# gvanhorn38/multibox

Measured on AMD Instinct MI355X. Metric: images/sec (299x299, 5-AR priors) train, higher is better.
Workload: dtype bf16; 1 GPU; full train step: Inception-ResNet-v2 + multibox heads fwd, on-device matching+loss, bwd, RMSProp+EMA; 299x299, k=5 (P=646), BATCH_SIZE=64/GPU, MAX_NUM_BBOXES=13; global_batch=64, parallelism=dp1, hip_graph=True

## Files before the change

multibox_amd/csrc/nnops.hip:

```cpp
#include "common.h"
#include <stdlib.h>
#include <string.h>

namespace {

__device__ __forceinline__ int xcd_logical(int bid, int nblk) {
  const int xcd = bid & 7, q = nblk >> 3, r = nblk & 7;
  return (xcd < r ? xcd * (q + 1) : r * (q + 1) + (xcd - r) * q) + (bid >> 3);
}
inline int xcd_rows_on() { static const int v = mbx_env_int("MBX_XCD_ROWS", 0); return v; }


typedef __attribute__((ext_vector_type(4))) unsigned int u32x4;
typedef __attribute__((ext_vector_type(2))) unsigned int u32x2;
constexpr int kT = 256;

__device__ __forceinline__ float bf2f(unsigned h) { return __uint_as_float(h << 16); }
__device__ __forceinline__ unsigned f2bf(float f) { return (unsigned)__builtin_bit_cast(unsigned short, (__bf16)f); }
__device__ __forceinline__ unsigned pack2bf(float lo, float hi) {
  typedef float pk_f32x2 __attribute__((ext_vector_type(2)));
  typedef __bf16 pk_bf16x2 __attribute__((ext_vector_type(2)));
  return __builtin_bit_cast(unsigned, __builtin_convertvector(pk_f32x2{lo, hi}, pk_bf16x2));
}
__device__ __forceinline__ float relu_f(float x) {
// ... 710 lines not shown
    const int e = threadIdx.x % C2, p = threadIdx.x / C2;
    float t[1];
    if (p < np) {
      ob_sum_cols<1, 16>(sred + p * C2 + e, 0, 1, np * C2, (rpi - p + np - 1) / np, t);
      part[p * C2 + e] = t[0];
    }
    __syncthreads();
    if (threadIdx.x < C2) {
      ob_sum_cols<1, 16>(part + threadIdx.x, 0, 1, C2, np, t);
      atomicAdd(acc + threadIdx.x, t[0]);
    }
  } else if (rpi > 8) ob_reduce_wide<1, 16>(sred, C2, rpi, acc);
  else if (rpi > 4) ob_reduce_wide<2, 8>(sred, C2, rpi, acc);
  else if (rpi > 2) ob_reduce_wide<4, 4>(sred, C2, rpi, acc);
  else if (rpi > 1) ob_reduce_wide<8, 2>(sred, C2, rpi, acc);
  else ob_reduce_wide<16, 1>(sred, C2, rpi, acc);
  asm volatile("s_waitcnt vmcnt(0) lgkmcnt(0)" ::: "memory");
  __syncthreads();
  if (threadIdx.x == 0) {
    const unsigned G = gridDim.x, b = blockIdx.x;
    const unsigned sub = b % kObSub, n_sub = (G - sub + kObSub - 1) / kObSub, n_top = G < kObSub ? G : kObSub;
    s_timeout = 0;
    bool last = ((fault & 1) && b == 0) ? false : atomicAdd(ctl + kObLine * (1 + sub), 1u) == n_sub - 1;
    if (last) last = atomicAdd(ctl + kObLine * (1 + kObSub), 1u) == n_top - 1;
    if (last) {
      for (int r = 0; r < kObRel; ++r)
        __hip_atomic_store(ctl + kObLine * (2 + kObSub + r), 1u, __ATOMIC_RELAXED, __HIP_MEMORY_SCOPE_AGENT);
    } else {
      const unsigned* rel = ctl + kObLine * (2 + kObSub + b % kObRel);
      unsigned spins = 0;
      while (ld_agent(rel) == 0u) {
        __builtin_amdgcn_s_sleep(MBX_OB_SLEEP);
        if (++spins > spin_limit) {
          ctl[1] = 1u; s_timeout = 1;
          if (step_poison) atomicAdd(step_poison, 1.0f);
          break;
        }
      }
    }
    if (b == 0) ctl[0] = G;
  }
  __syncthreads();
  for (int e = threadIdx.x; e < 2 * C; e += kObT) {
    float t = 0.f;
#pragma unroll
    for (int sl = 0; sl < kObSlots; ++sl) t += ld_agent(ws + (size_t)sl * 2 * C + e);
    sred[e] = t;
  }
  __syncthreads();
  float m1[8], m2[8], t1[8];
  const float poison = s_timeout ? __builtin_nanf("") : 0.f;
  {
    const float* tot = sred + (active ? c : 0);
    u32x4 p0 = *reinterpret_cast<const u32x4*>(tot), p1 = *reinterpret_cast<const u32x4*>(tot + 4);
    u32x4 q0 = *reinterpret_cast<const u32x4*>(tot + C), q1 = *reinterpret_cast<const u32x4*>(tot + C + 4);
    asm volatile("" : "+v"(p0), "+v"(p1), "+v"(q0), "+v"(q1));
#pragma unroll
    for (int j = 0; j < 4; ++j) {
      t1[j] = __uint_as_float(p0[j]); t1[4 + j] = __uint_as_float(p1[j]);
      m2[j] = __uint_as_float(q0[j]); m2[4 + j] = __uint_as_float(q1[j]);
    }
  }
#pragma unroll
  for (int j = 0; j < 8; ++j) {
    t1[j] = (active ? t1[j] : 0.f) + poison;
    m1[j] = t1[j] * inv_M;
    m2[j] = (active ? m2[j] : 0.f) * inv_M;
  }
  if (blockIdx.x == 0 && rr == 0 && dbeta) {
#pragma unroll
    for (int j = 0; j < 8; ++j) atomicAdd(dbeta + c + j, t1[j]);
  }
#pragma unroll
  for (int i = 0; i < NV; ++i) {
    const int lr = rr + i * rpi;
    const bool ok = active && lr < nrows;
    asm volatile("" : "+v"(vg[i]), "+v"(vy[i]));
    float g[8], yy[8], o[8];
    unpack8(vg[i], g);
    unpack8(vy[i], yy);
#pragma unroll
    for (int j = 0; j < 8; ++j) {
      const float xh = (yy[j] - mu[j]) * rs[j];
      const float gj = (!RELU || xh + be[j] > 0.f) ? g[j] : 0.f;
      o[j] = rs[j] * (gj - m1[j] - xh * m2[j]);
    }
    ob_store16(dr, ok ? (unsigned)((lr * C + c) * 2) : kPast, pack8(o));
    asm volatile("" ::: "memory");
  }
}

template <int KK, int SS>
__global__ void __launch_bounds__(kT)
maxpool_fwd_kernel(const unsigned short* __restrict__ x, long long xs, int ldx, int N, int H, int W, int C, int k_,
                   int stride_, unsigned short* __restrict__ y, long long ys, int ldy, int Ho, int Wo,
                   unsigned char* __restrict__ argmax) {
  const int k = KK ? KK : k_, stride = SS ? SS : stride_;
  const int C8 = C >> 3;
  const unsigned total = (unsigned)N * Ho * Wo * C8;
  for (unsigned i = blockIdx.x * kT + threadIdx.x; i < total; i += gridDim.x * kT) {
    unsigned t = i / (unsigned)C8;
    const int c = (int)(i - t * C8) << 3;
    const unsigned t2 = t / (unsigned)Wo;
    const int ow = (int)(t - t2 * Wo);
    const int n = (int)(t2 / (unsigned)Ho);
    const int oh = (int)(t2 - (unsigned)n * Ho);
    float best[8];
    unsigned arg[8];
#pragma unroll
    for (int j = 0; j < 8; ++j) { best[j] = -INFINITY; arg[j] = 0; }
    if constexpr (KK > 0) {
      u32x4 v[KK * KK];
#pragma unroll
      for (int r = 0; r < KK; ++r)
#pragma unroll
        for (int s = 0; s < KK; ++s) {
          const int h = oh * stride + r, w = ow * stride + s;
          v[r * KK + s] = (h < H && w < W) ? ld8(x + n * xs + ((long long)h * W + w) * ldx + c) : u32x4{0u, 0u, 0u, 0u};
        }
#pragma unroll
      for (int r = 0; r < KK; ++r)
#pragma unroll
        for (int s = 0; s < KK; ++s) {
          const int h = oh * stride + r, w = ow * stride + s;
          if (h >= H || w >= W) continue;
          float f[8];
          unpack8(v[r * KK + s], f);
#pragma unroll
          for (int j = 0; j < 8; ++j)
            if (f[j] > best[j]) { best[j] = f[j]; arg[j] = r * KK + s; }
        }
    } else {
      for (int r = 0; r < k; ++r)
        for (int s = 0; s < k; ++s) {
          const int h = oh * stride + r, w = ow * stride + s;
          if (h >= H || w >= W) continue;
          float f[8];
          unpack8(ld8(x + n * xs + ((long long)h * W + w) * ldx + c), f);
#pragma unroll
          for (int j = 0; j < 8; ++j)
            if (f[j] > best[j]) { best[j] = f[j]; arg[j] = r * k + s; }
        }
    }
    st8(y + n * ys + ((long long)oh * Wo + ow) * ldy + c, pack8(best));
    if (argmax) {
      u32x2 av;
      av.x = arg[0] | (arg[1] << 8) | (arg[2] << 16) | (arg[3] << 24);
      av.y = arg[4] | (arg[5] << 8) | (arg[6] << 16) | (arg[7] << 24);
      *reinterpret_cast<u32x2*>(argmax + (((long long)n * Ho + oh) * Wo + ow) * C + c) = av;
    }
  }
}

__global__ void __launch_bounds__(kT)
bn_apply_maxpool3s2_kernel(const unsigned short* __restrict__ y, int N, int H, int W, int C, const float* __restrict__ mean,
                           const float* __restrict__ rstd, const float* __restrict__ beta, int relu,
                           unsigned short* __restrict__ p, long long ps, int ldp, int Ho, int Wo,
                           unsigned char* __restrict__ argmax) {
  const int C8 = C >> 3;
  const unsigned total = (unsigned)N * Ho * Wo * C8;
  for (unsigned i = blockIdx.x * kT + threadIdx.x; i < total; i += gridDim.x * kT) {
    unsigned t = i / (unsigned)C8;
    const int c = (int)(i - t * C8) << 3;
    const unsigned t2 = t / (unsigned)Wo;
    const int ow = (int)(t - t2 * Wo);
    const int n = (int)(t2 / (unsigned)Ho);
    const int oh = (int)(t2 - (unsigned)n * Ho);
    u32x4 v[9];
#pragma unroll
    for (int r = 0; r < 3; ++r)
#pragma unroll
      for (int q = 0; q < 3; ++q)
        v[r * 3 + q] = ld8(y + (((long long)n * H + (oh * 2 + r)) * W + (ow * 2 + q)) * C + c);
    float mu[8], rs[8], be[8], best[8];
    unsigned arg[8];
#pragma unroll
    for (int j = 0; j < 8; ++j) { mu[j] = mean[c + j]; rs[j] = rstd[c + j]; be[j] = beta[c + j]; best[j] = -INFINITY; arg[j] = 0; }
#pragma unroll
    for (int tq = 0; tq < 9; ++tq) {
      float f[8];
      unpack8(v[tq], f);
#pragma unroll
      for (int j = 0; j < 8; ++j) {
        float a = (f[j] - mu[j]) * rs[j] + be[j];
        a = relu ? relu_f(a) : a;
        a = bf2f(f2bf(a));
        if (a > best[j]) { best[j] = a; arg[j] = tq; }
      }
    }
    st8(p + n * ps + ((long long)oh * Wo + ow) * ldp + c, pack8(best));
    if (argmax) {
      u32x2 av;
      av.x = arg[0] | (arg[1] << 8) | (arg[2] << 16) | (arg[3] << 24);
      av.y = arg[4] | (arg[5] << 8) | (arg[6] << 16) | (arg[7] << 24);
      *reinterpret_cast<u32x2*>(argmax + (((long long)n * Ho + oh) * Wo + ow) * C + c) = av;
    }
  }
}

struct PoolSrc { const unsigned short* gy; long long gys; int ld_gy; const unsigned char* argmax; int H, W, Ho, Wo, C, Hb, Wb; };
__device__ __forceinline__ void pool3s2_grad_block(const PoolSrc& p, int n, int a, int b, int c, float (&g)[4][8]) {
  u32x4 gv[4];
  u32x2 av[4];
  bool ok[4];
#pragma unroll
  for (int i = 0; i < 4; ++i) {
    const int oh = a - 1 + (i >> 1), ow = b - 1 + (i & 1);
    const bool v = oh >= 0 && oh < p.Ho && ow >= 0 && ow < p.Wo;
    ok[i] = v;
    const long long o = ((long long)n * p.Ho + (v ? oh : 0)) * p.Wo + (v ? ow : 0);
    av[i] = v ? *reinterpret_cast<const u32x2*>(p.argmax + o * p.C + c) : u32x2{0xffffffffu, 0xffffffffu};
    gv[i] = v ? ld8(p.gy + n * p.gys + ((long long)oh * p.Wo + ow) * p.ld_gy + c) : u32x4{0u, 0u, 0u, 0u};
  }
  float w[4][8];
#pragma unroll
  for (int i = 0; i < 4; ++i) unpack8(gv[i], w[i]);
  (void)ok;
#pragma unroll
  for (int j = 0; j < 8; ++j) {
    unsigned t[4];
#pragma unroll
    for (int i = 0; i < 4; ++i) t[i] = ((j < 4 ? av[i].x : av[i].y) >> (8 * (j & 3))) & 0xffu;
    float p00 = 0.f, p01 = 0.f, p10 = 0.f, p11 = 0.f;
    if (t[0] == 8u) p00 += w[0][j];
    if (t[1] == 6u) p00 += w[1][j];
    if (t[2] == 2u) p00 += w[2][j];
    if (t[3] == 0u) p00 += w[3][j];
    if (t[1] == 7u) p01 += w[1][j];
    if (t[3] == 1u) p01 += w[3][j];
    if (t[2] == 5u) p10 += w[2][j];
    if (t[3] == 3u) p10 += w[3][j];
    if (t[3] == 4u) p11 += w[3][j];
    g[0][j] = bf2f(f2bf(p00)); g[1][j] = bf2f(f2bf(p01)); g[2][j] = bf2f(f2bf(p10)); g[3][j] = bf2f(f2bf(p11));
  }
}

template <bool RELU>
__global__ void __launch_bounds__(kT)
bn_bwd_reduce_pool_kernel(const PoolSrc ps, const unsigned short* __restrict__ y, long long Mb, int C,
                          const float* __restrict__ mean, const float* __restrict__ rstd, const float* __restrict__ beta,
                          int rpi, int rpb, float* __restrict__ partial) {
  extern __shared__ __attribute__((aligned(16))) float sred[];
  const int C8 = C >> 3;
  const int vc = threadIdx.x % C8, rr = threadIdx.x / C8;
  const bool active = rr < rpi;
  const int c = vc << 3;
  float s1[8], s2[8], mu[8], rs[8], be[8];
#pragma unroll
  for (int j = 0; j < 8; ++j) {
    s1[j] = 0.f; s2[j] = 0.f; mu[j] = mean[c + j]; rs[j] = rstd[c + j];
    be[j] = RELU ? beta[c + j] : 0.f;
  }
  const long long r0 = (long long)blockIdx.x * rpb;
  long long r1 = r0 + rpb;
  if (r1 > Mb) r1 = Mb;
  const unsigned HWb = (unsigned)(ps.Hb * ps.Wb);
  if (active)
    for (long long m = r0 + rr; m < r1; m += rpi) {
      const unsigned mu_ = (unsigned)m, n = mu_ / HWb, rem = mu_ - n * HWb, a = rem / (unsigned)ps.Wb, b = rem - a * (unsigned)ps.Wb;
      u32x4 yv[4];
      bool in[4];
#pragma unroll
      for (int q = 0; q < 4; ++q) {
        const int h = 2 * (int)a + (q >> 1), w = 2 * (int)b + (q & 1);
        in[q] = h < ps.H && w < ps.W;
        yv[q] = ld8(y + (((long long)n * ps.H + (h < ps.H ? h : ps.H - 1)) * ps.W + (w < ps.W ? w : ps.W - 1)) * C + c);
      }
      float g[4][8];
      pool3s2_grad_block(ps, (int)n, (int)a, (int)b, c, g);
#pragma unroll
      for (int q = 0; q < 4; ++q) {
        float yy[8];
        unpack8(yv[q], yy);
#pragma unroll
        for (int j = 0; j < 8; ++j) {
          const float xh = (yy[j] - mu[j]) * rs[j];
          const float gj = (in[q] && (!RELU || xh + be[j] > 0.f)) ? g[q][j] : 0.f;
          s1[j] += gj;
          s2[j] += gj * xh;
        }
      }
    }
  if (active) {
    float* o = sred + ((size_t)rr * C8 + vc) * 16;
#pragma unroll
    for (int j = 0; j < 8; ++j) { o[j] = s1[j]; o[8 + j] = s2[j]; }
  }
  __syncthreads();
  if (threadIdx.x < C8) {
#pragma unroll
    for (int j = 0; j < 8; ++j) { s1[j] = 0.f; s2[j] = 0.f; }
    for (int r = 0; r < rpi; ++r) {
      const float* o = sred + ((size_t)r * C8 + threadIdx.x) * 16;
#pragma unroll
      for (int j = 0; j < 8; ++j) { s1[j] += o[j]; s2[j] += o[8 + j]; }
    }
    float* p = partial + ((size_t)blockIdx.x * C + (threadIdx.x << 3)) * 2;
#pragma unroll
    for (int j = 0; j < 8; ++j) { p[2 * j] = s1[j]; p[2 * j + 1] = s2[j]; }
  }
}

template <bool RELU>
__global__ void __launch_bounds__(kT)
bn_bwd_apply_pool_kernel(const PoolSrc ps, const unsigned short* __restrict__ y, long long Mb, int C, long long M,
                         const float* __restrict__ mean, const float* __restrict__ rstd, const float* __restrict__ beta,
                         const float* __restrict__ m12, unsigned short* __restrict__ dy) {
  const int C8 = C >> 3;
  const long long total = Mb * C8;
  const unsigned HWb = (unsigned)(ps.Hb * ps.Wb);
  for (long long i = (long long)blockIdx.x * kT + threadIdx.x; i < total; i += (long long)gridDim.x * kT) {
    const long long m = i / C8;
    const int c = (int)(i - m * C8) << 3;
    const unsigned mu_ = (unsigned)m, n = mu_ / HWb, rem = mu_ - n * HWb, a = rem / (unsigned)ps.Wb, b = rem - a * (unsigned)ps.Wb;
    float g[4][8], mu[8], rs[8], be[8], q1[8], q2[8];
#pragma unroll
    for (int j = 0; j < 8; ++j) {
      mu[j] = mean[c + j]; rs[j] = rstd[c + j]; be[j] = RELU ? beta[c + j] : 0.f; q1[j] = m12[c + j]; q2[j] = m12[C + c + j];
    }
    u32x4 yv[4];
#pragma unroll
    for (int q = 0; q < 4; ++q) {
      const int h = 2 * (int)a + (q >> 1), w = 2 * (int)b + (q & 1);
      yv[q] = ld8(y + (((long long)n * ps.H + (h < ps.H ? h : ps.H - 1)) * ps.W + (w < ps.W ? w : ps.W - 1)) * C + c);
    }
    pool3s2_grad_block(ps, (int)n, (int)a, (int)b, c, g);
#pragma unroll
    for (int q = 0; q < 4; ++q) {
      const int h = 2 * (int)a + (q >> 1), w = 2 * (int)b + (q & 1);
      if (h >= ps.H || w >= ps.W) continue;
      const long long row = ((long long)n * ps.H + h) * ps.W + w;
      float yy[8], o[8];
      unpack8(yv[q], yy);
#pragma unroll
      for (int j = 0; j < 8; ++j) {
        const float xh = (yy[j] - mu[j]) * rs[j];
        const float gj = (!RELU || xh + be[j] > 0.f) ? g[q][j] : 0.f;
        o[j] = rs[j] * (gj - q1[j] - xh * q2[j]);
      }
      st8(dy + row * C + c, pack8(o));
    }
  }
}

template <int KK, int SS>
__global__ void __launch_bounds__(kT)
maxpool_bwd_kernel(const unsigned short* __restrict__ dy, long long dys, int ld_dy,
                   const unsigned char* __restrict__ argmax, int N, int H, int W, int C, int k_, int stride_, int Ho,
// ... 581 lines not shown
extern "C" int mbx_bn_bwd_apply_mapped(const void* da, int ld_da, const void* a, int ld_a, int relu, const void* y, int64_t M,
                                       int C, const float* mean, const float* rstd, const float* beta, const float* m12,
                                       void* dy, const mbx_chan_map* da_map, mbx_stream_t stream) {
  if (!m12 || !dy || !al16(dy) || !bn_bwd_args_ok(da, ld_da, a, ld_a, relu, y, M, C, mean, rstd, beta))
    return MBX_ERR_INVALID_ARG;
  ChanMap cm;
  if (to_chan_map(da_map, C, cm) != MBX_OK || (da_map && da_map->n && a)) return MBX_ERR_INVALID_ARG;
  MBX_ENTER();
#define MBX_BN_APP(MASK)                                                                                            \
  hipLaunchKernelGGL(bn_bwd_apply_kernel<MASK>, dim3(grid_for(M * (C / 8))), dim3(kT), 0, mbx_s(stream), (cus)da,   \
                     ld_da, (cus)a, ld_a, (cus)y, (long long)M, C, mean, rstd, beta, m12, (us)dy, cm)
  if (!relu) MBX_BN_APP(0); else if (a) MBX_BN_APP(1); else MBX_BN_APP(2);
#undef MBX_BN_APP
  MBX_LAUNCH_CHECK();
  return MBX_OK;
}

extern "C" int mbx_bn_bwd_apply_rows(const float* stats, int rows, const void* da, int ld_da, const void* y, int64_t M, int C,
                                     const float* mean, const float* rstd, const float* relu_thr, float* dbeta, void* dy,
                                     const mbx_chan_map* da_map, mbx_stream_t stream) {
  if (!stats || rows <= 0 || rows > 16 || !da || !y || !mean || !rstd || !relu_thr || !dy || M <= 0 || C <= 0 || C % 8 ||
      ld_da % 8 || !al16(da) || !al16(y) || !al16(dy) || !al16(stats))
    return MBX_ERR_INVALID_ARG;
  if (C > kRowsMaxC) return MBX_ERR_UNSUPPORTED;
  ChanMap cm;
  if (to_chan_map(da_map, C, cm) != MBX_OK) return MBX_ERR_INVALID_ARG;
  MBX_ENTER();
  static const int rows_blocks = mbx_env_int("MBX_BN_ROWS_BLOCKS", 1024);
  const int C8 = C / 8, rpi = kT / C8 > 0 ? kT / C8 : 1;
  long long g = (M + rpi - 1) / rpi;
  if (g > rows_blocks) g = rows_blocks;
  hipLaunchKernelGGL(bn_bwd_rows_kernel, dim3((unsigned)g), dim3(kT), (size_t)5 * C * sizeof(float), mbx_s(stream), stats, rows,
                     1.0 / (double)M, (cus)da, ld_da, (cus)y, (long long)M, C, mean, rstd, relu_thr, dbeta, (us)dy, cm);
  MBX_LAUNCH_CHECK();
  return MBX_OK;
}

extern "C" size_t mbx_bn_bwd_onepass_workspace_bytes(int C) {
  return C > 0 ? ((size_t)kObSlots * 2 * C + kObCtlWords) * sizeof(float) : 0;
}

static int ob_groups(int max_workgroups) {
  const int ncu = mbx_cu_count();
  return (max_workgroups > 0 && max_workgroups < ncu) ? max_workgroups : ncu;
}

extern "C" int mbx_bn_bwd_onepass_supported(int64_t M, int C, int max_workgroups) {
  if (M <= 0 || C <= 0 || C % 8) return 0;
  const int ncu = ob_groups(max_workgroups);
  if (ncu <= 0) return 0;
  return ob_geom(M, C, ncu).nv <= kObMaxNV;
}

extern "C" int mbx_bn_bwd_onepass(const void* da, int ld_da, int relu, const void* y, int64_t M, int C, const float* mean,
                                  const float* rstd, const float* beta, float* dbeta, void* dy, void* ws,
                                  int max_workgroups, float* step_poison, mbx_stream_t stream) {
  return mbx_bn_bwd_onepass_mapped(da, ld_da, relu, y, M, C, mean, rstd, beta, dbeta, dy, ws, max_workgroups, step_poison,
                                   nullptr, stream);
}

extern "C" int mbx_bn_bwd_onepass_mapped(const void* da, int ld_da, int relu, const void* y, int64_t M, int C,
                                         const float* mean, const float* rstd, const float* beta, float* dbeta, void* dy,
                                         void* ws, int max_workgroups, float* step_poison, const mbx_chan_map* da_map,
                                         mbx_stream_t stream) {
  ChanMap cm;
  if (C <= 0 || to_chan_map(da_map, C, cm) != MBX_OK) return MBX_ERR_INVALID_ARG;
  const int map_max = chan_map_max(cm);
  if (!da || !y || !mean || !rstd || (relu && !beta) || !dy || !ws || M <= 0 || C <= 0 || C % 8 || ld_da % 8 || !al16(da) ||
      !al16(y) || !al16(dy) || !al16(ws) || !al16(mean) || !al16(rstd) || (relu && !al16(beta)))
    return MBX_ERR_INVALID_ARG;
  const int ncu = ob_groups(max_workgroups);
  if (ncu <= 0) return MBX_ERR_LAUNCH;
  const ObGeom g = ob_geom(M, C, ncu);
  if (g.nv > kObMaxNV) return MBX_ERR_UNSUPPORTED;
  MBX_ENTER();
  const size_t lds = ((size_t)g.rpi * 2 * C + (size_t)(2 * C > kObT ? 2 * C : kObT)) * sizeof(float);
  const int fault = mbx_barrier_fault() == '1';
  const unsigned spin_limit = fault ? (1u << 10) : (1u << 22);
#define MBX_OB(NV, RELU)                                                                                               \
  hipLaunchKernelGGL((bn_bwd_onepass_kernel<NV, RELU>), dim3(g.G), dim3(kObT), lds, mbx_s(stream), (cus)da, ld_da,      \
                     (cus)y, (long long)M, C, mean, rstd, beta, dbeta, (us)dy, (float*)ws, g.rpi, g.rpb,               \
                     (float)(1.0 / (double)M), spin_limit, fault | (xcd_rows_on() << 1), step_poison, cm, map_max)
#define MBX_OB_NV(NV) do { if (relu) MBX_OB(NV, true); else MBX_OB(NV, false); } while (0)
  if (g.nv <= 2) MBX_OB_NV(2);
  else if (g.nv <= 4) MBX_OB_NV(4);
  else if (g.nv <= 8) MBX_OB_NV(8);
  else if (g.nv <= 12) MBX_OB_NV(12);
  else if (g.nv <= 16) MBX_OB_NV(16);
  else MBX_OB_NV(20);
#undef MBX_OB_NV
#undef MBX_OB
  MBX_LAUNCH_CHECK();
  return MBX_OK;
}

static int pool_args_ok(const void* x, int ldx, const void* y, int ldy, int N, int H, int W, int C, int k, int Ho, int Wo) {
  return x && y && N > 0 && H > 0 && W > 0 && C > 0 && C % 8 == 0 && ldx % 8 == 0 && ldy % 8 == 0 && k > 0 && k < 16 &&
         Ho > 0 && Wo > 0 && al16(x) && al16(y) && (long long)N * H * W * (C / 8) < (1LL << 31) &&
         (long long)N * Ho * Wo * (C / 8) < (1LL << 31);
}

extern "C" int mbx_maxpool_fwd(const void* x, int64_t xs, int ldx, int N, int H, int W, int C, int k, int stride, void* y,
                               int64_t ys, int ldy, int Ho, int Wo, uint8_t* argmax, mbx_stream_t stream) {
  if (!pool_args_ok(x, ldx, y, ldy, N, H, W, C, k, Ho, Wo) || stride < 1) return MBX_ERR_INVALID_ARG;
  if ((Ho - 1) * stride + k > H || (Wo - 1) * stride + k > W) return MBX_ERR_INVALID_ARG;
  MBX_ENTER();
  if (k == 3 && stride == 2)
    hipLaunchKernelGGL((maxpool_fwd_kernel<3, 2>), dim3(grid_for((long long)N * Ho * Wo * (C / 8))), dim3(kT), 0, mbx_s(stream),
                       (cus)x, (long long)xs, ldx, N, H, W, C, k, stride, (us)y, (long long)ys, ldy, Ho, Wo, argmax);
  else
    hipLaunchKernelGGL((maxpool_fwd_kernel<0, 0>), dim3(grid_for((long long)N * Ho * Wo * (C / 8))), dim3(kT), 0, mbx_s(stream),
                       (cus)x, (long long)xs, ldx, N, H, W, C, k, stride, (us)y, (long long)ys, ldy, Ho, Wo, argmax);
  MBX_LAUNCH_CHECK();
  return MBX_OK;
}

extern "C" int mbx_maxpool_bwd(const void* dy, int64_t dys, int ld_dy, const uint8_t* argmax, int N, int H, int W, int C,
                               int k, int stride, int Ho, int Wo, void* dx, int64_t dxs, int ld_dx, int accumulate,
                               mbx_stream_t stream) {
  if (!pool_args_ok(dy, ld_dy, dx, ld_dx, N, H, W, C, k, Ho, Wo) || !argmax || stride < 1) return MBX_ERR_INVALID_ARG;
  MBX_ENTER();
  if (k == 3 && stride == 2)
    hipLaunchKernelGGL((maxpool_bwd_kernel<3, 2>), dim3(grid_for((long long)N * H * W * (C / 8))), dim3(kT), 0, mbx_s(stream),
                       (cus)dy, (long long)dys, ld_dy, argmax, N, H, W, C, k, stride, Ho, Wo, (us)dx, (long long)dxs, ld_dx,
                       accumulate);
  else
    hipLaunchKernelGGL((maxpool_bwd_kernel<0, 0>), dim3(grid_for((long long)N * H * W * (C / 8))), dim3(kT), 0, mbx_s(stream),
                       (cus)dy, (long long)dys, ld_dy, argmax, N, H, W, C, k, stride, Ho, Wo, (us)dx, (long long)dxs, ld_dx,
                       accumulate);
  MBX_LAUNCH_CHECK();
  return MBX_OK;
}

static int pool_src_ok(const void* gy, int ld_gy, const uint8_t* argmax, int N, int H, int W, int Ho, int Wo, int C, PoolSrc& ps,
                       int64_t gys) {
  if (!gy || !argmax || N <= 0 || H <= 0 || W <= 0 || C <= 0 || C % 8 || ld_gy % 8 || !al16(gy) || (reinterpret_cast<uintptr_t>(argmax) & 7))
    return MBX_ERR_INVALID_ARG;
  if (Ho != (H - 3) / 2 + 1 || Wo != (W - 3) / 2 + 1) return MBX_ERR_INVALID_ARG;
  if ((long long)N * H * W >= (1LL << 31)) return MBX_ERR_UNSUPPORTED;
  ps.gy = (cus)gy; ps.gys = gys; ps.ld_gy = ld_gy; ps.argmax = argmax; ps.H = H; ps.W = W; ps.Ho = Ho; ps.Wo = Wo; ps.C = C;
  ps.Hb = (H + 1) / 2; ps.Wb = (W + 1) / 2;
  return MBX_OK;
}

extern "C" int mbx_bn_apply_maxpool(const void* y, int N, int H, int W, int C, const float* mean, const float* rstd,
                                    const float* beta, int relu, void* p, int64_t p_img_stride, int ld_p, int Ho, int Wo,
                                    uint8_t* argmax, mbx_stream_t stream) {
  if (!y || !p || !mean || !rstd || !beta || N <= 0 || H < 3 || W < 3 || C <= 0 || C % 8 || ld_p % 8 || !al16(y) || !al16(p) ||
      (argmax && (reinterpret_cast<uintptr_t>(argmax) & 7)))
    return MBX_ERR_INVALID_ARG;
  if (Ho != (H - 3) / 2 + 1 || Wo != (W - 3) / 2 + 1) return MBX_ERR_INVALID_ARG;
  if ((long long)N * Ho * Wo * (C / 8) >= (1LL << 31) || (long long)N * H * W * C >= (1LL << 40)) return MBX_ERR_UNSUPPORTED;
  MBX_ENTER();
  hipLaunchKernelGGL(bn_apply_maxpool3s2_kernel, dim3(grid_for((long long)N * Ho * Wo * (C / 8))), dim3(kT), 0, mbx_s(stream),
                     (cus)y, N, H, W, C, mean, rstd, beta, relu, (us)p, (long long)p_img_stride, ld_p, Ho, Wo, argmax);
  MBX_LAUNCH_CHECK();
  return MBX_OK;
}

extern "C" int mbx_bn_bwd_rows_pooled(int N, int H, int W, int C) {
  if (N <= 0 || H <= 0 || W <= 0 || C <= 0 || C % 8 || C > 2048) return MBX_ERR_INVALID_ARG;
  return bn_bwd_geom((long long)N * ((H + 1) / 2) * ((W + 1) / 2), C).rows;
}

extern "C" int mbx_bn_bwd_reduce_pooled(const void* gy, int64_t gy_img_stride, int ld_gy, const uint8_t* argmax, int N, int H,
                                        int W, int Ho, int Wo, int relu, const void* y, int C, const float* mean,
                                        const float* rstd, const float* beta, float* partial, mbx_stream_t stream) {
  PoolSrc ps;
  int st = pool_src_ok(gy, ld_gy, argmax, N, H, W, Ho, Wo, C, ps, gy_img_stride);
  if (st != MBX_OK) return st;
  if (!y || !al16(y) || !mean || !rstd || (relu && !beta) || !partial || C > 2048) return MBX_ERR_INVALID_ARG;
  const long long Mb = (long long)N * ps.Hb * ps.Wb;
  const BnBwdGeom g = bn_bwd_geom(Mb, C);
  MBX_ENTER();
  const size_t lds = (size_t)g.rows_per_iter * g.C8 * 16 * sizeof(float);
  if (relu)
    hipLaunchKernelGGL(bn_bwd_reduce_pool_kernel<true>, dim3(g.rows), dim3(kT), lds, mbx_s(stream), ps, (cus)y, Mb, C, mean, rstd,
                       beta, g.rows_per_iter, g.rpb, partial);
  else
    hipLaunchKernelGGL(bn_bwd_reduce_pool_kernel<false>, dim3(g.rows), dim3(kT), lds, mbx_s(stream), ps, (cus)y, Mb, C, mean, rstd,
                       beta, g.rows_per_iter, g.rpb, partial);
  MBX_LAUNCH_CHECK();
  return MBX_OK;
}

extern "C" int mbx_bn_bwd_apply_pooled(const void* gy, int64_t gy_img_stride, int ld_gy, const uint8_t* argmax, int N, int H,
                                       int W, int Ho, int Wo, int relu, const void* y, int C, const float* mean,
                                       const float* rstd, const float* beta, const float* m12, void* dy, mbx_stream_t stream) {
  PoolSrc ps;
  int st = pool_src_ok(gy, ld_gy, argmax, N, H, W, Ho, Wo, C, ps, gy_img_stride);
  if (st != MBX_OK) return st;
  if (!y || !al16(y) || !mean || !rstd || (relu && !beta) || !m12 || !dy || !al16(dy)) return MBX_ERR_INVALID_ARG;
  const long long M = (long long)N * H * W, Mb = (long long)N * ps.Hb * ps.Wb;
  MBX_ENTER();
  if (relu)
    hipLaunchKernelGGL(bn_bwd_apply_pool_kernel<true>, dim3(grid_for(Mb * (C / 8))), dim3(kT), 0, mbx_s(stream), ps, (cus)y, Mb, C, M,
                       mean, rstd, beta, m12, (us)dy);
  else
    hipLaunchKernelGGL(bn_bwd_apply_pool_kernel<false>, dim3(grid_for(Mb * (C / 8))), dim3(kT), 0, mbx_s(stream), ps, (cus)y, Mb, C, M,
                       mean, rstd, beta, m12, (us)dy);
  MBX_LAUNCH_CHECK();
  return MBX_OK;
}

extern "C" int mbx_avgpool_fwd(const void* x, int64_t xs, int ldx, int N, int H, int W, int C, int k, int pad, void* y,
                               int64_t ys, int ldy, int Ho, int Wo, mbx_stream_t stream) {
  if (!pool_args_ok(x, ldx, y, ldy, N, H, W, C, k, Ho, Wo) || pad < 0 || pad >= k) return MBX_ERR_INVALID_ARG;
  if (Ho != H + 2 * pad - k + 1 || Wo != W + 2 * pad - k + 1) return MBX_ERR_INVALID_ARG;
  MBX_ENTER();
  hipLaunchKernelGGL(avgpool_fwd_kernel, dim3(grid_for((long long)N * Ho * Wo * (C / 8))), dim3(kT), 0, mbx_s(stream),
                     (cus)x, (long long)xs, ldx, N, H, W, C, k, pad, (us)y, (long long)ys, ldy, Ho, Wo);
  MBX_LAUNCH_CHECK();
  return MBX_OK;
}

extern "C" int mbx_avgpool_bwd(const void* dy, int64_t dys, int ld_dy, int N, int H, int W, int C, int k, int pad, int Ho,
                               int Wo, void* dx, int64_t dxs, int ld_dx, int accumulate, mbx_stream_t stream) {
  if (!pool_args_ok(dy, ld_dy, dx, ld_dx, N, H, W, C, k, Ho, Wo) || pad < 0 || pad >= k) return MBX_ERR_INVALID_ARG;
  MBX_ENTER();
  hipLaunchKernelGGL(avgpool_bwd_kernel, dim3(grid_for((long long)N * H * W * (C / 8))), dim3(kT), 0, mbx_s(stream),
                     (cus)dy, (long long)dys, ld_dy, N, H, W, C, k, pad, Ho, Wo, (us)dx, (long long)dxs, ld_dx, accumulate);
  MBX_LAUNCH_CHECK();
  return MBX_OK;
}

extern "C" int mbx_relu_mask(void* g, int ld_g, const void* a, int ld_a, int64_t M, int C, mbx_stream_t stream) {
  if (!g || !a || M <= 0 || C <= 0 || C % 8 || ld_g % 8 || ld_a % 8 || !al16(g) || !al16(a)) return MBX_ERR_INVALID_ARG;
  MBX_ENTER();
  hipLaunchKernelGGL(relu_mask_kernel, dim3(grid_for(M * (C / 8))), dim3(kT), 0, mbx_s(stream), (us)g, ld_g, (cus)a, ld_a,
                     (long long)M, C);
  MBX_LAUNCH_CHECK();
  return MBX_OK;
}

extern "C" int mbx_pack_input(const float* img, int64_t pixels, void* out, mbx_stream_t stream) {
  if (!img || !out || pixels <= 0 || !al16(out)) return MBX_ERR_INVALID_ARG;
  MBX_ENTER();
  hipLaunchKernelGGL(pack_input_kernel, dim3(grid_for(pixels)), dim3(kT), 0, mbx_s(stream), img, (long long)pixels, (us)out);
  MBX_LAUNCH_CHECK();
  return MBX_OK;
}

extern "C" int mbx_head_gather(const float* h, int ld_h, int N, int cells, int k, int P, int off, float* locs,
                               float* logits, mbx_stream_t stream) {
  if (!h || !locs || !logits || N <= 0 || cells <= 0 || k <= 0 || ld_h < 5 * k || off < 0 || off + cells * k > P)
    return MBX_ERR_INVALID_ARG;
  MBX_ENTER();
  hipLaunchKernelGGL(head_gather_kernel, dim3(grid_for((long long)N * cells * k)), dim3(kT), 0, mbx_s(stream), h, ld_h, N,
                     cells, k, P, off, locs, logits);
  MBX_LAUNCH_CHECK();
  return MBX_OK;
}

extern "C" int mbx_head_scatter(const float* d_locs, const float* d_logits, int N, int cells, int k, int P, int off, void* g,
                                int ld_g, mbx_stream_t stream) {
  if (!d_locs || !d_logits || !g || N <= 0 || cells <= 0 || k <= 0 || ld_g < 5 * k || off < 0 || off + cells * k > P)
    return MBX_ERR_INVALID_ARG;
  MBX_ENTER();
  hipLaunchKernelGGL(head_scatter_kernel, dim3(grid_for((long long)N * cells * ld_g)), dim3(kT), 0, mbx_s(stream), d_locs,
                     d_logits, N, cells, k, P, off, (us)g, ld_g);
  MBX_LAUNCH_CHECK();
  return MBX_OK;
}

static int fill_head_table(const mbx_head* heads, int n_heads, int N, int P, bool scatter, HeadTable& t) {
  if (!heads || n_heads <= 0 || n_heads > kMaxHeads || N <= 0 || P <= 0) return MBX_ERR_INVALID_ARG;
  long long acc = 0;
  t.n = n_heads;
  for (int j = 0; j < n_heads; ++j) {
    const mbx_head& H = heads[j];
    if (H.cells <= 0 || H.k <= 0 || H.off < 0 || H.off + H.cells * H.k > P) return MBX_ERR_INVALID_ARG;
    if (scatter ? (!H.g || H.ld_g < 5 * H.k) : (!H.h || H.ld_h < 5 * H.k)) return MBX_ERR_INVALID_ARG;
    t.h[j] = H.h; t.g[j] = reinterpret_cast<unsigned short*>(H.g);
    t.ld_h[j] = H.ld_h; t.ld_g[j] = H.ld_g; t.cells[j] = H.cells; t.k[j] = H.k; t.off[j] = H.off;
    t.start[j] = (int)acc;
    acc += (long long)N * H.cells * (scatter ? H.ld_g : H.k);
    if (acc >= (1LL << 31)) return MBX_ERR_UNSUPPORTED;
  }
  for (int j = n_heads; j <= kMaxHeads; ++j) t.start[j] = (int)acc;
  return MBX_OK;
}

extern "C" int mbx_head_gather_all(const mbx_head* heads, int n_heads, int N, int P, float* locs, float* logits,
                                   mbx_stream_t stream) {
  if (!locs || !logits) return MBX_ERR_INVALID_ARG;
  HeadTable t;
  const int st = fill_head_table(heads, n_heads, N, P, false, t);
  if (st != MBX_OK) return st;
  MBX_ENTER();
  hipLaunchKernelGGL(head_gather_all_kernel, dim3(grid_for(t.start[t.n])), dim3(kT), 0, mbx_s(stream), t, P, locs, logits);
  MBX_LAUNCH_CHECK();
  return MBX_OK;
}

extern "C" int mbx_head_scatter_all(const float* d_locs, const float* d_logits, const mbx_head* heads, int n_heads, int N,
                                    int P, mbx_stream_t stream) {
  if (!d_locs || !d_logits) return MBX_ERR_INVALID_ARG;
  HeadTable t;
  const int st = fill_head_table(heads, n_heads, N, P, true, t);
  if (st != MBX_OK) return st;
  MBX_ENTER();
  hipLaunchKernelGGL(head_scatter_all_kernel, dim3(grid_for(t.start[t.n])), dim3(kT), 0, mbx_s(stream), t, P, d_locs, d_logits);
  MBX_LAUNCH_CHECK();
  return MBX_OK;
}

extern "C" int mbx_step_begin(float* grads, int64_t n_grads, float* bn_ws, int64_t n_ws, int64_t ctl_index,
                              uint64_t* timeouts_total, float* zero_scalar, mbx_stream_t stream) {
// ... 99 lines not shown
```

Measured before the change: 4422 images/sec.

## Tile fused BN+maxpool3s2 into patches reusing overlapping rows and columns

Rewrites the fused BN-apply + 3x3 stride-2 maxpool kernel so each thread handles a patch of 2 output columns by up to 6 output rows for one 8-channel group. Shared input columns and rows are loaded once and the BN is applied once, with the bottom row scan carried into the next output row and the following rows prefetched. This targets the roughly 2.25x redundant loads and BN math of the per-output approach. The relu flag becomes a template parameter. In exchange the kernel uses more registers, exposes less parallelism per launch, and has a more complex edge-clamping path.

```diff
diff --git a/multibox_amd/csrc/nnops.hip b/multibox_amd/csrc/nnops.hip
--- a/multibox_amd/csrc/nnops.hip
+++ b/multibox_amd/csrc/nnops.hip
@@ -886,48 +886,110 @@
   }
 }
 
+constexpr int kPoolPW = 2, kPoolPH = 6;
+template <int PW>
+struct PoolRowScan { float m[PW][8]; unsigned t[PW][8]; };
+
+template <int PW, bool RELU>
+__device__ __forceinline__ void pool3s2_scan_row(const u32x4 (&v)[2 * PW + 1], const float (&mu)[8], const float (&rs)[8],
+                                                 const float (&be)[8], PoolRowScan<PW>& s) {
+#pragma unroll
+  for (int o = 0; o < PW; ++o)
+#pragma unroll
+    for (int j = 0; j < 8; ++j) { s.m[o][j] = -INFINITY; s.t[o][j] = 0u; }
+#pragma unroll
+  for (int q = 0; q < 2 * PW + 1; ++q) {
+    float f[8];
+    unpack8(v[q], f);
+#pragma unroll
+    for (int j = 0; j < 8; ++j) {
+      float a = (f[j] - mu[j]) * rs[j] + be[j];
+      a = RELU ? relu_f(a) : a;
+      f[j] = bf2f(f2bf(a));
+    }
+#pragma unroll
+    for (int o = 0; o < PW; ++o) {
+      const int t = q - 2 * o;
+      if (t < 0 || t > 2) continue;
+#pragma unroll
+      for (int j = 0; j < 8; ++j)
+        if (f[j] > s.m[o][j]) { s.m[o][j] = f[j]; s.t[o][j] = (unsigned)t; }
+    }
+  }
+}
+
+template <int PW, bool RELU>
 __global__ void __launch_bounds__(kT)
 bn_apply_maxpool3s2_kernel(const unsigned short* __restrict__ y, int N, int H, int W, int C, const float* __restrict__ mean,
-                           const float* __restrict__ rstd, const float* __restrict__ beta, int relu,
+                           const float* __restrict__ rstd, const float* __restrict__ beta,
                            unsigned short* __restrict__ p, long long ps, int ldp, int Ho, int Wo,
-                           unsigned char* __restrict__ argmax) {
+                           unsigned char* __restrict__ argmax, int ph) {
+  constexpr int NQ = 2 * PW + 1;
   const int C8 = C >> 3;
-  const unsigned total = (unsigned)N * Ho * Wo * C8;
-  for (unsigned i = blockIdx.x * kT + threadIdx.x; i < total; i += gridDim.x * kT) {
-    unsigned t = i / (unsigned)C8;
-    const int c = (int)(i - t * C8) << 3;
-    const unsigned t2 = t / (unsigned)Wo;
-    const int ow = (int)(t - t2 * Wo);
-    const int n = (int)(t2 / (unsigned)Ho);
-    const int oh = (int)(t2 - (unsigned)n * Ho);
-    u32x4 v[9];
-#pragma unroll
-    for (int r = 0; r < 3; ++r)
-#pragma unroll
-      for (int q = 0; q < 3; ++q)
-        v[r * 3 + q] = ld8(y + (((long long)n * H + (oh * 2 + r)) * W + (ow * 2 + q)) * C + c);
-    float mu[8], rs[8], be[8], best[8];
-    unsigned arg[8];
-#pragma unroll
-    for (int j = 0; j < 8; ++j) { mu[j] = mean[c + j]; rs[j] = rstd[c + j]; be[j] = beta[c + j]; best[j] = -INFINITY; arg[j] = 0; }
-#pragma unroll
-    for (int tq = 0; tq < 9; ++tq) {
-      float f[8];
-      unpack8(v[tq], f);
-#pragma unroll
-      for (int j = 0; j < 8; ++j) {
-        float a = (f[j] - mu[j]) * rs[j] + be[j];
-        a = relu ? relu_f(a) : a;
-        a = bf2f(f2bf(a));
-        if (a > best[j]) { best[j] = a; arg[j] = tq; }
+  const int cw = C8 < kT ? C8 : kT;
+  const int rpi = kT / cw;
+  const int vc = (int)blockIdx.y * cw + (int)threadIdx.x % cw, rr = (int)threadIdx.x / cw;
+  if (rr >= rpi || vc >= C8) return;
+  const int c = vc << 3;
+  float mu[8], rs[8], be[8];
+#pragma unroll
+  for (int j = 0; j < 8; ++j) { mu[j] = mean[c + j]; rs[j] = rstd[c + j]; be[j] = beta[c + j]; }
+  const unsigned Wp = (unsigned)(Wo + PW - 1) / PW, S = (unsigned)(Ho + ph - 1) / ph;
+  const unsigned npatch = (unsigned)N * S * Wp;
+  const long long row = (long long)W * C;
+  for (unsigned pi = blockIdx.x * rpi + rr; pi < npatch; pi += gridDim.x * rpi) {
+    const unsigned t1 = pi / Wp, n = t1 / S;
+    const int ow0 = (int)(pi - t1 * Wp) * PW, oh0 = (int)(t1 - n * S) * ph;
+    const int oh1 = oh0 + ph < Ho ? oh0 + ph : Ho;
+    int qo[NQ];
+#pragma unroll
+    for (int q = 0; q < NQ; ++q) qo[q] = (2 * ow0 + q < W ? q : W - 1 - 2 * ow0) * C;
+    const unsigned short* yr = y + (((long long)n * H + 2 * oh0) * W + 2 * ow0) * C + c;
+    u32x4 top[NQ], cur[2][NQ];
+#pragma unroll
+    for (int q = 0; q < NQ; ++q) { top[q] = ld8(yr + qo[q]); cur[0][q] = ld8(yr + row + qo[q]); cur[1][q] = ld8(yr + 2 * row + qo[q]); }
+    PoolRowScan<PW> carry;
+    pool3s2_scan_row<PW, RELU>(top, mu, rs, be, carry);
+    unsigned short* po = p + n * ps + ((long long)oh0 * Wo + ow0) * ldp + c;
+    unsigned char* ao = argmax ? argmax + (((long long)n * Ho + oh0) * Wo + ow0) * C + c : nullptr;
+    for (int oh = oh0; oh < oh1; ++oh) {
+      yr += 2 * row;
+      u32x4 nxt[2][NQ];
+      if (oh + 1 < oh1) {
+#pragma unroll
+        for (int q = 0; q < NQ; ++q) { nxt[0][q] = ld8(yr + row + qo[q]); nxt[1][q] = ld8(yr + 2 * row + qo[q]); }
+      } else {
+#pragma unroll
+        for (int q = 0; q < NQ; ++q) { nxt[0][q] = cur[0][q]; nxt[1][q] = cur[1][q]; }
       }
-    }
-    st8(p + n * ps + ((long long)oh * Wo + ow) * ldp + c, pack8(best));
-    if (argmax) {
-      u32x2 av;
-      av.x = arg[0] | (arg[1] << 8) | (arg[2] << 16) | (arg[3] << 24);
-      av.y = arg[4] | (arg[5] << 8) | (arg[6] << 16) | (arg[7] << 24);
-      *reinterpret_cast<u32x2*>(argmax + (((long long)n * Ho + oh) * Wo + ow) * C + c) = av;
+      PoolRowScan<PW> mid, bot;
+      pool3s2_scan_row<PW, RELU>(cur[0], mu, rs, be, mid);
+      pool3s2_scan_row<PW, RELU>(cur[1], mu, rs, be, bot);
+#pragma unroll
+      for (int o = 0; o < PW; ++o) {
+        float best[8];
+        unsigned arg[8];
+#pragma unroll
+        for (int j = 0; j < 8; ++j) {
+          best[j] = carry.m[o][j]; arg[j] = carry.t[o][j];
+          if (mid.m[o][j] > best[j]) { best[j] = mid.m[o][j]; arg[j] = 3u + mid.t[o][j]; }
+          if (bot.m[o][j] > best[j]) { best[j] = bot.m[o][j]; arg[j] = 6u + bot.t[o][j]; }
+        }
+        if (ow0 + o < Wo) {
+          st8(po + o * ldp, pack8(best));
+          if (ao) {
+            u32x2 av;
+            av.x = arg[0] | (arg[1] << 8) | (arg[2] << 16) | (arg[3] << 24);
+            av.y = arg[4] | (arg[5] << 8) | (arg[6] << 16) | (arg[7] << 24);
+            *reinterpret_cast<u32x2*>(ao + o * C) = av;
+          }
+        }
+      }
+      carry = bot;
+      po += (long long)Wo * ldp;
+      if (ao) ao += (long long)Wo * C;
+#pragma unroll
+      for (int q = 0; q < NQ; ++q) { cur[0][q] = nxt[0][q]; cur[1][q] = nxt[1][q]; }
     }
   }
 }
@@ -1815,8 +1877,15 @@
   if (Ho != (H - 3) / 2 + 1 || Wo != (W - 3) / 2 + 1) return MBX_ERR_INVALID_ARG;
   if ((long long)N * Ho * Wo * (C / 8) >= (1LL << 31) || (long long)N * H * W * C >= (1LL << 40)) return MBX_ERR_UNSUPPORTED;
   MBX_ENTER();
-  hipLaunchKernelGGL(bn_apply_maxpool3s2_kernel, dim3(grid_for((long long)N * Ho * Wo * (C / 8))), dim3(kT), 0, mbx_s(stream),
-                     (cus)y, N, H, W, C, mean, rstd, beta, relu, (us)p, (long long)p_img_stride, ld_p, Ho, Wo, argmax);
+  const int C8 = C / 8, cw = C8 < kT ? C8 : kT, rpi = kT / cw;
+  const long long npatch = (long long)N * ((Ho + kPoolPH - 1) / kPoolPH) * ((Wo + kPoolPW - 1) / kPoolPW);
+  const dim3 grid(grid_for((npatch + rpi - 1) / rpi * kT), (C8 + cw - 1) / cw);
+  if (relu)
+    hipLaunchKernelGGL((bn_apply_maxpool3s2_kernel<kPoolPW, true>), grid, dim3(kT), 0, mbx_s(stream), (cus)y, N, H, W, C, mean, rstd,
+                       beta, (us)p, (long long)p_img_stride, ld_p, Ho, Wo, argmax, kPoolPH);
+  else
+    hipLaunchKernelGGL((bn_apply_maxpool3s2_kernel<kPoolPW, false>), grid, dim3(kT), 0, mbx_s(stream), (cus)y, N, H, W, C, mean, rstd,
+                       beta, (us)p, (long long)p_img_stride, ld_p, Ho, Wo, argmax, kPoolPH);
   MBX_LAUNCH_CHECK();
   return MBX_OK;
 }
```

Result: no change. 4427 images/sec, median of 6 (+0.1%).
